# facebookresearch/any4

Measured on AMD Instinct MI355X. Metric: any4 W4A16 GEMM achieved GB/s (m=1, n=k=4096, g=128), higher is better.
Workload: dtype bf16

## Files before the change

any4_amd/csrc/tg_common.cuh:

```cuda
#pragma once
#include <hip/hip_runtime.h>
#include <stdint.h>
#include <stdlib.h>
#include <string.h>
#include <atomic>
#include <type_traits>
#include <utility>

#include "../../include/tinygemm_hip.h"
#include "tg_trace.cuh"

struct GemmParams {
  const char* x;
  const char* w;
  const char* qinfo;
  const char* lut;
  char* y;
  int32_t m, wrows, k;
  int32_t ntiles;
  int32_t ksuper;
  int32_t gshift;
  int32_t ngroups;
  int32_t qtype;
  int32_t rowtiles;
// ... 144 lines not shown

struct BF16 {
  static __device__ __forceinline__ float to_f32(uint16_t h) { return u2f(((uint32_t)h) << 16); }
  static __device__ __forceinline__ float lo_f32(uint32_t pair) { return u2f(pair << 16); }
  static __device__ __forceinline__ float hi_f32(uint32_t pair) { return u2f(pair & 0xffff0000u); }
  static __device__ __forceinline__ uint32_t pack2(float a, float b) {
    f32x2 v = {a, b};
    return __builtin_bit_cast(uint32_t, __builtin_convertvector(v, bf16x2));
  }
  static __device__ __forceinline__ uint16_t from_f32(float a) { return (uint16_t)(pack2(a, 0.f) & 0xffffu); }
  static __device__ __forceinline__ f32x4 mfma(u32x4 a, u32x4 b, f32x4 c) {
    return __builtin_amdgcn_mfma_f32_16x16x32_bf16(__builtin_bit_cast(bf16x8, a), __builtin_bit_cast(bf16x8, b), c, 0, 0, 0);
  }
};
struct F16 {
  static __device__ __forceinline__ float to_f32(uint16_t h) { return (float)__builtin_bit_cast(_Float16, h); }
  static __device__ __forceinline__ float lo_f32(uint32_t pair) { return to_f32((uint16_t)(pair & 0xffffu)); }
  static __device__ __forceinline__ float hi_f32(uint32_t pair) { return to_f32((uint16_t)(pair >> 16)); }
  static __device__ __forceinline__ uint32_t pack2(float a, float b) {
    f32x2 v = {a, b};
    return __builtin_bit_cast(uint32_t, __builtin_convertvector(v, f16x2));
  }
  static __device__ __forceinline__ uint16_t from_f32(float a) { return (uint16_t)(pack2(a, 0.f) & 0xffffu); }
  static __device__ __forceinline__ f32x4 mfma(u32x4 a, u32x4 b, f32x4 c) {
    return __builtin_amdgcn_mfma_f32_16x16x32_f16(__builtin_bit_cast(f16x8, a), __builtin_bit_cast(f16x8, b), c, 0, 0, 0);
  }
};

template <int... VS, typename F>
int pick(int v, F&& f) {
  int rc = TG_PAIR_NA;
  (void)((v == VS && ((rc = f(std::integral_constant<int, VS>{})), true)) || ...);
  return rc;
}
template <typename F>
int pick_dt(int dt, F&& f) {
  return dt == TG_BF16 ? f(BF16{}) : f(F16{});
}

__device__ const float kMX4Values[16] = {0.0f,  0.5f,  1.0f,  1.5f,  2.0f,  3.0f,  4.0f,  6.0f,
                                         -0.0f, -0.5f, -1.0f, -1.5f, -2.0f, -3.0f, -4.0f, -6.0f};

template <typename DT>
__device__ __forceinline__ void store_rows4(char* yb, const char* bias, int64_t elem, int rowg, f32x4 acc) {
  u32x2 o = {DT::pack2(acc[0], acc[1]), DT::pack2(acc[2], acc[3])};
  if (bias) {
    const u32x2 bv = *reinterpret_cast<const u32x2*>(bias + (int64_t)rowg * 2);
    o[0] = DT::pack2(DT::lo_f32(o[0]) + DT::lo_f32(bv[0]), DT::hi_f32(o[0]) + DT::hi_f32(bv[0]));
    o[1] = DT::pack2(DT::lo_f32(o[1]) + DT::lo_f32(bv[1]), DT::hi_f32(o[1]) + DT::hi_f32(bv[1]));
  }
  *reinterpret_cast<u32x2*>(yb + elem * 2) = o;
}


__device__ __forceinline__ u32x4 transpose_rows4(u32x4 v) {
  const auto s01 = __builtin_amdgcn_permlane16_swap(v[0], v[1], false, false);
  const auto s23 = __builtin_amdgcn_permlane16_swap(v[2], v[3], false, false);
  const auto t02 = __builtin_amdgcn_permlane32_swap(s01[0], s23[0], false, false);
  const auto t13 = __builtin_amdgcn_permlane32_swap(s01[1], s23[1], false, false);
  return u32x4{t02[0], t13[0], t02[1], t13[1]};
}

struct DeviceScope {
  int prev = -1;
  bool ok = true;
  explicit DeviceScope(int device) {
    if (device < 0) return;
    if (hipGetDevice(&prev) != hipSuccess) { ok = false; return; }
    if (prev != device && hipSetDevice(device) != hipSuccess) ok = false;
    if (prev == device) prev = -1;
  }
  ~DeviceScope() {
    if (prev >= 0) (void)hipSetDevice(prev);
  }
};

inline int launch_status() {
  const hipError_t e = hipGetLastError();
  return e == hipSuccess ? 0 : (int)e;
}

inline bool aligned16(const void* p) { return (reinterpret_cast<uintptr_t>(p) & 15u) == 0; }
inline int64_t cdiv(int64_t a, int64_t b) { return (a + b - 1) / b; }
inline int group_shift(int g) { return g == 32 ? 5 : g == 64 ? 6 : g == 128 ? 7 : 8; }
inline int64_t coltiles(const GemmParams& p) { return cdiv(p.m, 16); }
inline int words_per_lane(const GemmParams& p) { return p.on_right ? p.inner / 2 : p.inner; }

template <typename D, typename F>
auto assign_if_member(D& d, F f, int) -> decltype(f(d)) { f(d); }
template <typename D, typename F>
void assign_if_member(D&, F, long) {}
template <typename D>
void copy_call(D& d, const GemmParams& p) {
#define TG_COPY(f) assign_if_member(d, [&](auto& t) -> decltype((void)(t.f = p.f)) { t.f = p.f; }, 0)
  TG_COPY(x); TG_COPY(w); TG_COPY(qinfo); TG_COPY(lut); TG_COPY(y);
  TG_COPY(m); TG_COPY(wrows); TG_COPY(k); TG_COPY(ntiles); TG_COPY(ksuper); TG_COPY(gshift); TG_COPY(ngroups); TG_COPY(qtype);
  TG_COPY(stride_x); TG_COPY(stride_w); TG_COPY(stride_qinfo); TG_COPY(stride_lut); TG_COPY(stride_y);
  TG_COPY(bias); TG_COPY(stride_bias); TG_COPY(bias_row_stride);
  TG_COPY(norm_w); TG_COPY(norm_eps); TG_COPY(epilogue); TG_COPY(x_tc); TG_COPY(y_tc); TG_COPY(dry);
#undef TG_COPY
}
inline SplitKParams splitk_params(const GemmParams& p, int splitk) {
  SplitKParams kp;
  copy_call(kp, p);
  kp.rowtiles = p.rowtiles;
  kp.splitk = splitk;
  kp.sk_shift = 0;
  while ((1 << kp.sk_shift) < splitk) ++kp.sk_shift;
  return kp;
}

inline bool has_workspace(const GemmParams& p, int64_t need) { return p.ws_query || (p.ws != nullptr && p.ws_bytes >= need); }

template <auto KERN>
int prepare_lds_kernel() {
  static std::atomic<uint64_t> done{0};
  int dev = 0;
  if (hipGetDevice(&dev) != hipSuccess) return TG_E_DEVICE;
  if (dev >= 0 && dev < 64 && ((done.load(std::memory_order_relaxed) >> dev) & 1u)) return 0;
  hipFuncAttributes fa;
  hipError_t e = hipFuncGetAttributes(&fa, reinterpret_cast<const void*>(KERN));
  if (e != hipSuccess) return (int)e;
  if (fa.sharedSizeBytes != 0) return TG_E_INTERNAL;
  e = hipFuncSetAttribute(reinterpret_cast<const void*>(KERN), hipFuncAttributeMaxDynamicSharedMemorySize, 160 * 1024);
  if (e != hipSuccess) return (int)e;
  if (dev >= 0 && dev < 64) done.fetch_or(1ull << dev, std::memory_order_relaxed);
  return 0;
}
template <auto KERN, typename P>
int launch_lds_kernel(dim3 grid, dim3 block, unsigned lds, hipStream_t st, const P& params, bool decline_on_failure) {
  const int prc = prepare_lds_kernel<KERN>();
  if (prc != 0) return decline_on_failure && prc != TG_E_INTERNAL ? (int)TG_PAIR_NA : prc;
  hipLaunchKernelGGL(KERN, grid, block, lds, st, params);
  return launch_status();
}

inline int cu_count() {
  static std::atomic<int> cache[64];
  int dev = 0;
  if (hipGetDevice(&dev) != hipSuccess || dev < 0 || dev >= 64) return 256;
  int v = cache[dev].load(std::memory_order_relaxed);
  if (v > 0) return v;
  if (hipDeviceGetAttribute(&v, hipDeviceAttributeMultiprocessorCount, dev) != hipSuccess || v <= 0) v = 256;
  cache[dev].store(v, std::memory_order_relaxed);
  return v;
}
inline int plan_cu_count(const GemmParams& p) { return p.dry ? 256 : cu_count(); }


#if !defined(TG_DEV) && !defined(TG_DEV_MIN)
#if defined(TG_PAIR_R) || defined(TG_PAIR_MR1) || defined(TG_PAIR_NSG2) || defined(TG_PAIR_MR1_GPS) || defined(TG_PAIR_RA) ||   \
    defined(TG_PAIR_RA1) || defined(TG_PAIR_RB16) || defined(TG_B16_CHUNK) || defined(TG_PAIR_MIN_ITEMS) || defined(TG_XG_CHUNK) || defined(TG_PAIR_WGS) || \
    defined(TG_PAIR_NSG2_M1) || defined(TG_XR_MIN_M) || defined(TG_XR_R) || defined(TG_XR_R8K) || defined(TG_XR_RMX) || defined(TG_PAIR_M1_LEAN) || \
    defined(TG_PAIR_M1_AHEAD)
#error "the TG_PAIR_* / TG_XG_* / TG_B16_* tuning constants can only be overridden in developer builds (-DTG_DEV or -DTG_DEV_MIN)"
#endif
#endif
#ifndef TG_PAIR_R
#define TG_PAIR_R 2
#endif
#ifndef TG_PAIR_MR1
#define TG_PAIR_MR1 1
#endif
#ifndef TG_PAIR_NSG2
#define TG_PAIR_NSG2 1
#endif
#ifndef TG_PAIR_NSG2_M1
#define TG_PAIR_NSG2_M1 1
#endif
#ifndef TG_PAIR_MR1_GPS
#define TG_PAIR_MR1_GPS 1
#endif
#ifndef TG_PAIR_RA
#define TG_PAIR_RA 2
#endif
#ifndef TG_PAIR_RA1
#define TG_PAIR_RA1 1
#endif
#ifndef TG_PAIR_RB16
#define TG_PAIR_RB16 2
#endif
#ifndef TG_B16_CHUNK
#define TG_B16_CHUNK 4
#endif
#ifndef TG_TILE_W8_MIN_M
#define TG_TILE_W8_MIN_M 17
#endif
#ifndef TG_TILE_MIN_M_SPLIT
#define TG_TILE_MIN_M_SPLIT 17
#endif
#ifndef TG_TILE_MIN_M
#define TG_TILE_MIN_M 65
#endif
#ifndef TG_M1_DEFAULT_MFMA
#define TG_M1_DEFAULT_MFMA 0
#endif
#ifndef TG_PAIR_MIN_ITEMS
#define TG_PAIR_MIN_ITEMS 192
#endif
#ifndef TG_XG_CHUNK
#define TG_XG_CHUNK 4
#endif
#ifndef TG_XR_MIN_M
#define TG_XR_MIN_M 2
#endif
#ifndef TG_XR_RMX
#define TG_XR_RMX 8
#endif
#ifndef TG_XR_R8K
#define TG_XR_R8K 2
#endif
#ifndef TG_XR_R
#define TG_XR_R 4
#endif
#ifndef TG_PAIR_M1_LEAN
#define TG_PAIR_M1_LEAN 1
#endif
#ifndef TG_PAIR_M1_AHEAD
#define TG_PAIR_M1_AHEAD 1
#endif
#ifndef TG_PAIR_WGS
#define TG_PAIR_WGS 512
#endif

}
```

any4_amd/csrc/tg_pair.hip:

```cpp
#include "tg_common.cuh"
#ifdef TG_TU_F16
#define TG_TU_DT F16
#define TG_TU_SUF(n) n##_f16
#else
#define TG_TU_DT BF16
#define TG_TU_SUF(n) n##_bf16
#endif
namespace {
#include "w4_gemm_pair.cuh"
template <typename DT, int I, int GPS, int MR, bool QMX, int NSG, bool XG = false, int LA = 0, bool NORM = false, bool M1_MFMA = false>
int launch_pair_k(const GemmParams& p, PairParams& pp, unsigned lds) {
#ifdef TG_DEV_MIN
#ifndef TG_DEV_GPS
#define TG_DEV_GPS 1
#endif
#ifndef TG_DEV_QMX
#define TG_DEV_QMX false
#endif
#ifndef TG_DEV_MR
#define TG_DEV_MR TG_PAIR_MR1
#endif
#ifndef TG_DEV_LA
#define TG_DEV_LA 0
#endif
  if constexpr (!(std::is_same<DT, BF16>::value && I == 4 && GPS == TG_DEV_GPS && MR == TG_DEV_MR && QMX == TG_DEV_QMX && NSG == TG_DEV_MIN && LA == TG_DEV_LA && !NORM)) return TG_PAIR_NA;
  else {
#endif
  if constexpr (QMX && !std::is_same<DT, BF16>::value) return TG_E_DTYPE;
  else {
  constexpr int RING = (QMX && LA == 0) ? TG_PAIR_R : (MR == 1 && NSG == 4 && LA == 0) ? 4 : GPS > 1 ? (LA ? TG_PAIR_RA1 : 1) : LA == 1 ? TG_PAIR_RA : LA == 2 ? TG_PAIR_RB16 : TG_PAIR_R;
  if (p.dry) return TG_PLAN_PAIR;
  const unsigned wgs = (unsigned)(pp.items < TG_PAIR_WGS ? pp.items : TG_PAIR_WGS);
  return launch_lds_kernel<w4_gemm_pair_kernel<DT, I, GPS, MR, QMX, RING, NSG, M1_MFMA, XG, LA, NORM>>(dim3(wgs), dim3(512), lds, p.st, pp, false);
  }
#ifdef TG_DEV_MIN
  }
#endif
}

inline bool pair_lean_call(const GemmParams& p, const PairParams& pp, bool xg) {
  return TG_PAIR_M1_LEAN && TG_PAIR_MR1 == 1 && TG_PAIR_R == 2 && p.m == 1 && !xg && !p.norm_w && !p.bias && !p.epilogue && !p.x_tc && !p.y_tc &&
         p.wrows % 64 == 0 && p.ntiles * 8 == p.wrows && !pp.red_alias && pp.cblocks == 1 && pp.spw % 2 == 0 && p.ksuper % 2 == 0 &&
         p.numerics != TG_NUM_FAST_MFMA;
}
template <typename DT>
int launch_pair_lean(const GemmParams& p, const PairParams& pp, unsigned lds) {
#ifdef TG_DEV_MIN
  if constexpr (!(std::is_same<DT, BF16>::value && TG_DEV_MIN == 2)) return TG_PAIR_NA;
  else {
#endif
  if (p.dry) return p.dry_detail ? (int)TG_PLAN_PAIR_M1_LEAN : (int)TG_PLAN_PAIR;
  PairLeanParams lp;
  copy_call(lp, p);
  lp.spw = pp.spw; lp.lds_x = pp.lds_x; lp.lds_xs = pp.lds_xs; lp.lds_red = pp.lds_red; lp.rblocks = pp.rblocks; lp.items = pp.items;
  const unsigned wgs = (unsigned)(pp.items < TG_PAIR_WGS ? pp.items : TG_PAIR_WGS);
  return launch_lds_kernel<w4_pair_m1_lean_kernel<DT, TG_PAIR_M1_AHEAD != 0>>(dim3(wgs), dim3(512), lds, p.st, lp, false);
#ifdef TG_DEV_MIN
  }
#endif
}

template <typename DT>
int launch_xprep(const GemmParams& p, const PairParams& pp, int ma, int la = 0) {
  XPrepParams xq;
  xq.la = la;
  xq.x = pp.x; xq.xp = const_cast<char*>(pp.xp); xq.xsum = const_cast<char*>(pp.xsum);
  xq.x_tc = pp.x_tc;
  xq.m = pp.m; xq.k = pp.k; xq.ma = ma; xq.cps = p.inner / 2; xq.gshift = pp.gshift; xq.gch_mask = pp.gch_mask;
  xq.ngroups = pp.ngroups; xq.xs_rows = pp.xs_rows;
  xq.stride_x = pp.stride_x; xq.stride_xp = pp.stride_xp; xq.stride_xsum = pp.stride_xsum;
  const int64_t chunks = (int64_t)pp.m * (pp.k / 32);
  hipLaunchKernelGGL(w4_xprep_kernel<DT>, dim3((unsigned)cdiv(chunks, 256), (unsigned)p.batch), dim3(256), 0, p.st, xq);
  return launch_status();
}

template <typename DT, int I, int GPS, bool QMX, int NSG>
int launch_pair_m(const GemmParams& p, PairParams& pp, unsigned lds, bool xg, int mregs) {
  const bool norm = p.norm_w != nullptr;
  const bool m1 = p.m == 1 && TG_PAIR_MR1 == 1 && (QMX || GPS <= TG_PAIR_MR1_GPS);
  if (mregs != 4) return TG_PAIR_NA;
  if constexpr (I == 8) {
    if constexpr (QMX) return TG_PAIR_NA;
    else {
      if (!m1 || norm) return TG_PAIR_NA;
      return xg ? launch_pair_k<DT, I, GPS, 1, false, NSG, true>(p, pp, lds) : launch_pair_k<DT, I, GPS, 1, false, NSG>(p, pp, lds);
    }
  } else {
  if (xg) return m1 ? launch_pair_k<DT, I, GPS, 1, QMX, NSG, true>(p, pp, lds) : launch_pair_k<DT, I, GPS, 4, QMX, NSG, true>(p, pp, lds);
  if (norm) {
    if constexpr (QMX || GPS > 1) return TG_PAIR_NA;
    else {
      return m1 ? launch_pair_k<DT, I, GPS, 1, false, NSG, false, false, true>(p, pp, lds)
                : launch_pair_k<DT, I, GPS, 4, false, NSG, false, false, true>(p, pp, lds);
    }
  }
  if (m1) return launch_pair_k<DT, I, GPS, 1, QMX, NSG>(p, pp, lds);
  return launch_pair_k<DT, I, GPS, 4, QMX, NSG>(p, pp, lds);
  }
}


struct PairGroups {
  int gps, nsg;
};
template <int I>
PairGroups pair_groups(const GemmParams& p, PairParams& pp) {
  const int g = 1 << p.gshift;
  const PairGroups r = {g >= 16 * I ? 1 : (16 * I) / g, g >= 16 * I ? g / (16 * I) : 1};
  const int units = p.ksuper / r.nsg;
  pp.spw = ((units + 7) / 8) * r.nsg;
  pp.nsg_shift = 0;
  while ((1 << pp.nsg_shift) < r.nsg) ++pp.nsg_shift;
  pp.gch_mask = g / 32 - 1;
  return r;
}

inline bool mx4_blocks_fit(const GemmParams& p, const PairParams& pp, int gps) {
  return !(p.ngroups < 16 || p.ngroups % 4 != 0 || ((pp.spw * gps) % 4 != 0 && pp.spw * gps > 12));
}

template <int I, bool QMX>
unsigned pair_lds_plan(const GemmParams& p, PairParams& pp, int x_bytes, bool alias, bool alias_if_large) {
  pp.lds_x = QMX ? 0 : 65536;
  pp.lds_xs = (pp.lds_x + x_bytes + 32 * I + 15) & ~15;
  pp.lds_red = (pp.lds_xs + (QMX ? 0 : p.ngroups * pp.xs_rows * 4) + 15) & ~15;
  unsigned lds = (unsigned)pp.lds_red + (unsigned)(8 * 2 * pp.rused * pp.red_lanes * 4);
  pp.red_alias = alias || (alias_if_large && lds > 80u * 1024u);
  if (pp.red_alias) {
    lds = (unsigned)pp.lds_red;
    pp.lds_red = 0;
  }
  return lds;
}

inline int64_t pair_workspace(const GemmParams& p, PairParams& pp, int xrows) {
  pp.stride_xp = (int64_t)xrows * p.k * 2;
  pp.stride_xsum = ((int64_t)p.ngroups * pp.xs_rows * 4 + 15) & ~(int64_t)15;
  const int64_t need = p.batch * (pp.stride_xp + pp.stride_xsum);
  if (!has_workspace(p, need)) return 0;
  pp.xp = p.ws;
  pp.xsum = p.ws + p.batch * pp.stride_xp;
  return need;
}

template <typename DT, int I, bool QMX>
int launch_pair(GemmParams& p) {
  constexpr int RW = 64;
  const int mregs = p.m <= 8 ? 4 : 16;
  const int ma = 2 * mregs;
  PairParams pp;
  copy_call(pp, p);
  pp.y_tiles = (p.wrows + 15) / 16;
  const auto [gps, nsg] = pair_groups<I>(p, pp);
  const int mrows = p.m < ma ? p.m : ma;
  pp.rused = mrows < 4 ? mrows : mregs;
  pp.xs_rows = mrows <= 4 ? 4 : ma;
  pp.red_lanes = mrows <= 4 ? 32 : 64;
  pp.x_pitch = p.k * 2 + 16;
  unsigned lds = pair_lds_plan<I, QMX>(p, pp, mrows * pp.x_pitch, !QMX && mrows > 4, false);
  if (QMX && !mx4_blocks_fit(p, pp, gps)) return TG_PAIR_NA;
  if (p.norm_w && (QMX || lds > 80u * 1024u || p.m > ma)) return TG_PAIR_NA;
  int64_t need = 0;
  if (lds > 80u * 1024u) {
    if (mregs != 4 || p.m > ma) return TG_PAIR_NA;
    pp.xw_pitch = 32 * I + 16;
    pp.xw_bytes = (I == 2 ? 16 : 8) * pp.xw_pitch;
    lds = pair_lds_plan<I, QMX>(p, pp, 8 * pp.xw_bytes, pp.red_alias, true);
    if (QMX && pp.red_alias) return TG_PAIR_NA;
    if (lds > 80u * 1024u) return TG_PAIR_NA;
    need = pair_workspace(p, pp, p.m);
    if (!need) return TG_PAIR_NA;
  }
  const bool xg = need != 0;
  pp.rblocks = (p.wrows + RW - 1) / RW;
  pp.cblocks = (p.m + ma - 1) / ma;
  const int64_t items = (int64_t)pp.rblocks * pp.cblocks * p.batch;
  if (items > INT32_MAX) return TG_PAIR_NA;
  if (items < TG_PAIR_MIN_ITEMS) return TG_PAIR_NA;
  pp.items = (int32_t)items;
  pp.chunk = items >= (int64_t)TG_PAIR_WGS * TG_XG_CHUNK * 4 ? TG_XG_CHUNK : 1;
  p.ws_need = need;
  if (xg && !p.dry) {
    const int rc = launch_xprep<DT>(p, pp, ma);
    if (rc != 0) return rc;
  }
  if (gps == 1) {
    const bool fixed = TG_PAIR_NSG2 && (TG_PAIR_NSG2_M1 || !(p.m == 1 && TG_PAIR_MR1 == 1));
    if constexpr (I == 4 && !QMX) {
      if (p.numerics == TG_NUM_FAST_MFMA && p.m == 1 && !xg && !p.norm_w && fixed && nsg == TG_PAIR_R)
        return launch_pair_k<DT, I, 1, 1, false, TG_PAIR_R, false, 0, false, true>(p, pp, lds);
    }
    if constexpr (I == 4 && !QMX) {
      if (fixed && nsg == TG_PAIR_R && pair_lean_call(p, pp, xg)) return launch_pair_lean<DT>(p, pp, lds);
    }
    if (fixed && nsg == TG_PAIR_R) return launch_pair_m<DT, I, 1, QMX, TG_PAIR_R>(p, pp, lds, xg, mregs);
    if constexpr (!QMX) {
      if (fixed && p.m == 1 && TG_PAIR_MR1 == 1 && !p.norm_w && (nsg == 1 || nsg == 4)) {
        if (nsg == 1) return xg ? launch_pair_k<DT, I, 1, 1, false, 1, true>(p, pp, lds) : launch_pair_k<DT, I, 1, 1, false, 1>(p, pp, lds);
        if constexpr (I <= 4)
          return xg ? launch_pair_k<DT, I, 1, 1, false, 4, true>(p, pp, lds) : launch_pair_k<DT, I, 1, 1, false, 4>(p, pp, lds);
      }
    }
    return launch_pair_m<DT, I, 1, QMX, 0>(p, pp, lds, xg, mregs);
  }
  if constexpr (I >= 4) {
    if (gps == 2) return launch_pair_m<DT, I, 2, QMX, 0>(p, pp, lds, xg, mregs);
  }
  if constexpr (I >= 8) {
// ... 69 lines not shown
```

any4_amd/csrc/w4_gemm_pair.cuh:

```cuda
#pragma once
#include "w4_helpers.cuh"
#include "pair_walk.h"

struct PairParams {
  const char* x;
  const char* w;
  const char* qinfo;
  const char* lut;
  char* y;
  int32_t m, wrows, k;
  int32_t ntiles;
  int32_t ksuper;
  int32_t gshift;
  int32_t ngroups;
  int32_t qtype;
  int32_t spw;
  int32_t nsg_shift;
  int32_t gch_mask;
  int32_t x_pitch;
  int32_t lds_x;
  int32_t lds_xs;
  int32_t lds_red;
  int32_t rused;
  int32_t xs_rows;
  int32_t red_lanes;
  int32_t red_alias;
  int32_t rblocks;
  int32_t cblocks;
  int32_t items;
  int64_t stride_x, stride_w, stride_qinfo, stride_lut, stride_y;
  const char* bias;
  int64_t stride_bias;
  int64_t bias_row_stride;
  const char* norm_w;
  float norm_eps;
  int32_t epilogue;
  int32_t dry;
  const char* xp;
  const char* xsum;
  int64_t stride_xp, stride_xsum;
  int32_t xw_pitch;
  int32_t xw_bytes;
  int32_t chunk;
  int32_t x_tc, y_tc;
  int32_t y_tiles;
};

template <typename DT, int I, int GPS, int MR, bool QMX, int R, int NSG = 0, bool M1_MFMA = false, bool XG = false, int LAY = 0, bool NORM = false>
__global__ void __launch_bounds__(512, 4) w4_gemm_pair_kernel(const PairParams p) {
  constexpr bool LA = LAY == 1, LB = LAY == 2, T16 = LAY != 0;
  constexpr bool DOT = !M1_MFMA && MR == 1 && !T16 && (QMX || NSG > 0);
  constexpr bool MXC = QMX;
  static_assert(!NORM || (!XG && !T16 && !QMX), "fused RMSNorm: the workgroup stages the whole activation block itself");
  constexpr int WAVES = 8;
  constexpr int TILES = 2;
  constexpr int WT = LA ? 1 : TILES;
  constexpr int RW = T16 ? 32 : 32 * TILES;
  static_assert(!T16 || (XG && MR == 4 && (LB || I == 2 || I == 4)), "16x16x32 tiles: workspace activations, one pass of up to 16 rows");
  constexpr int NW = LB ? I / 2 : I;
  using acc_t = typename std::conditional<T16, f32x4, f32x16>::type;
  constexpr int CPS = I / 2;
  constexpr int CPG = CPS / GPS;
  constexpr int MREGS = MR == 1 ? 4 : MR;
  constexpr int RF = MR;
  constexpr int MA = T16 ? 16 : 2 * MREGS;
  constexpr int NXW = T16 ? I / 2 : XG ? (MA * 2 * I + 63) / 64 : 1;
  static_assert(!XG || MR <= 4, "XG: one pass is at most 8 activation rows");

  constexpr uint32_t lds0 = 0u;
  const uint32_t lds_x = lds0 + (uint32_t)p.lds_x;
  const uint32_t lds_xs = lds0 + (uint32_t)p.lds_xs;
  const uint32_t lds_red = lds0 + (uint32_t)p.lds_red;

  const int tid = threadIdx.x;
  const int lane = tid & 63;
  const int wave = __builtin_amdgcn_readfirstlane(tid >> 6);
  const int c = lane & 31;
  const int h = lane >> 5;
  const int xa = DOT ? 0 : T16 ? lane & 15 : c;
  const int xq = T16 ? lane >> 4 : 2 * h;
  const int hh = T16 ? lane >> 4 : h;
  auto wrow_local = [&](int t) -> int { return LA ? 16 * ((lane & 15) >> 3) + (lane & 7) + 8 * t : LB ? 16 * t + (lane & 15) : t * 32 + c; };
  const int tcol = tid & 63;
  const int tcol_row = LA ? 16 * ((tcol & 15) >> 3) + (tcol & 7) + 8 * (tcol >> 5) : LB ? 16 * (tcol >> 5) + (tcol & 15) : tcol;

  constexpr bool RR = XG;
  const int chunk = RR ? p.chunk : 1;
  const int it_stride = RR ? (int)gridDim.x * chunk - (chunk - 1) : 1;
  const int it_begin = RR ? (int)blockIdx.x * chunk : (int)(((int64_t)blockIdx.x * p.items) / gridDim.x);
  const int it_end = RR ? p.items : (int)(((int64_t)(blockIdx.x + 1) * p.items) / gridDim.x);
  const int per_problem = p.rblocks * p.cblocks;

  const int s_begin = wave * p.spw;
  const int nl = max(min(p.spw, p.ksuper - s_begin), 0);

  struct Item {
    int b, ct, rb;
  };
  auto decode = [&](int it) -> Item {
    const int b = it / per_problem, r = it - b * per_problem;
    const int ct = r / p.rblocks;
    return Item{b, ct, r - ct * p.rblocks};
  };
  const int adv_b = it_stride / per_problem, adv_r = it_stride - adv_b * per_problem;
  auto advance = [&](const Item& e, bool big) -> Item {
    int b = e.b + (big ? adv_b : 0), r = e.ct * p.rblocks + e.rb + (big ? adv_r : 1);
    if (r >= per_problem) { r -= per_problem; ++b; }
    const int ct = p.cblocks == 1 ? 0 : r / p.rblocks;
    return Item{b, ct, r - ct * p.rblocks};
  };

  uint32_t lp[8];
  auto lut_const = [&]() {
#pragma unroll
    for (int e = 0; e < 16; e += 2) {
      float v0, v1;
      if (p.qtype == TG_Q_INT4) {
        v0 = (float)(e - 8);
        v1 = (float)(e - 7);
      } else {
        const int e1 = e + 1;
        v0 = (e & 8 ? -1.f : 1.f) * ((e & 7) < 5 ? 0.5f * (e & 7) : ((e & 7) == 5 ? 3.f : (e & 7) == 6 ? 4.f : 6.f));
        v1 = (e1 & 8 ? -1.f : 1.f) * ((e1 & 7) < 5 ? 0.5f * (e1 & 7) : ((e1 & 7) == 5 ? 3.f : (e1 & 7) == 6 ? 4.f : 6.f));
      }
      lp[e >> 1] = DT::pack2(v0, v1);
    }
  };
  const bool lut_loaded = p.qtype == TG_Q_ANY4_GLOBAL || p.qtype == TG_Q_ANY4_ROWWISE;
  auto lut_request = [&](const Item& e) {
    const int lrow = min(e.rb * RW + tcol_row, p.wrows - 1);
    const char* lsrc = p.lut + (int64_t)e.b * p.stride_lut + (p.qtype == TG_Q_ANY4_ROWWISE ? (int64_t)lrow * 32 : 0);
    const u32x4 l0 = reinterpret_cast<const u32x4*>(lsrc)[0];
    const u32x4 l1 = reinterpret_cast<const u32x4*>(lsrc)[1];
#pragma unroll
    for (int j = 0; j < 4; ++j) { lp[j] = l0[j]; lp[4 + j] = l1[j]; }
  };

  struct Slot {
    uint32_t w[WT][I];
    uint32_t q[TILES][GPS];
    u32x4 xw[NXW];
  };
  Slot ring[R];
  struct Rows {
    uint32_t wbase[WT];
    uint32_t qrow[TILES];
    uint32_t qrow4[TILES];
    const char* wb;
    const char* qb;
    const char* xpb;
    uint32_t xblk;
    uint32_t xoff[NXW];
  };
  auto rows_of = [&](const Item& e) -> Rows {
    Rows r;
// ... 469 lines not shown
      }
    };

    const int rounds = max((nl + R - 1) / R, 1);
    int l0 = 0;
    const int nblk = QMX ? max((nl + EBS - 1) / EBS, 1) : 1;
    for (int blk = 0; blk < nblk; ++blk) {
      const bool lastb = blk + 1 == nblk;
      if constexpr (QMX) {
#pragma unroll
        for (int t = 0; t < TILES; ++t) ecur[t] = enext[t];
        ebase = eoff_next - blk * 16;
        e_request(lastb ? rnext : rcur, lastb ? 0 : blk + 1, lastb ? has_next && nl > 0 : true);
      }
      const int rend = lastb ? rounds - 1 : (blk + 1) * (EBS / R);
      for (int rd = l0 / R; rd < rend; ++rd, l0 += R) {
#pragma unroll
        for (int j = 0; j < R; ++j) {
          consume(s_begin + l0 + j, ring[j], j);
          issue(rcur, s_begin + l0 + j + R, ring[j], l0 + j + R < nl, NSG == 0 || j % NSG == 0);
        }
      }
    }
#pragma unroll
    for (int j = 0; j < R; ++j) {
      if (l0 + j < nl) consume(s_begin + l0 + j, ring[j], j);
      issue(rnext, s_begin + j, ring[j], has_next && j < nl, NSG == 0 || j % NSG == 0);
    }
    if constexpr (MXC) {
#pragma unroll
      for (int t = 0; t < TILES; ++t)
#pragma unroll
        for (int r = 0; r < RF; ++r) yacc[t][r] = DOT ? dacc[t] : acc[t][r];
    } else if (pending || GPS > 1 || NSG > 0) finalize();
    if constexpr (DOT) {
#pragma unroll
      for (int t = 0; t < TILES; ++t) yacc[t][0] += __shfl_xor(yacc[t][0], 32);
    }

    if (p.red_alias) __syncthreads();
#pragma unroll
    for (int t = 0; t < TILES; ++t) {
#pragma unroll
      for (int r = 0; r < RF; ++r)
        if (r < p.rused && lane < p.red_lanes)
          *(lds_fptr)(lds_red + (uint32_t)((((wave * TILES + t) * p.rused + r) * p.red_lanes + lane) * 4)) = yacc[t][r];
    }
    __syncthreads();
    {
      char* yb = p.y + (int64_t)cur.b * p.stride_y;
      static_assert(TILES == 2, "the output index split below assumes two tiles");
      const int rl_shift = p.red_lanes == 64 ? 6 : 5;
      for (int o = tid; o < TILES * p.rused * p.red_lanes; o += 512) {
        const int l = o & (p.red_lanes - 1), q = o >> rl_shift;
        const int t = q >= p.rused ? 1 : 0, r = q - t * p.rused;
        const int a = T16 ? r + 4 * (l >> 4) : (r & 3) + 8 * (r >> 2) + 4 * (l >> 5);
        const int row = row0 + (LA ? 16 * ((l & 15) >> 3) + (l & 7) + 8 * t : LB ? 16 * t + (l & 15) : t * 32 + (l & 31));
        if (a < mrows && row < p.wrows) {
          float sum = 0.f;
#pragma unroll
          for (int w = 0; w < WAVES; ++w) sum += *(lds_fptr)(lds_red + (uint32_t)((((w * TILES + t) * p.rused + r) * p.red_lanes + l) * 4));
          if (!T16 && p.epilogue == TG_EPI_SWIGLU) {
            if ((l & 15) < 8) {
              float up = 0.f;
#pragma unroll
              for (int w = 0; w < WAVES; ++w) up += *(lds_fptr)(lds_red + (uint32_t)((((w * TILES + t) * p.rused + r) * p.red_lanes + l + 8) * 4));
              *reinterpret_cast<uint16_t*>(yb + ((int64_t)(a0 + a) * (p.wrows >> 1) + ((row >> 4) << 3) + (row & 7)) * 2) = swiglu16<DT>(sum, up);
            }
            continue;
          }
          uint16_t o16 = DT::from_f32(sum);
          if (p.bias)
            o16 = DT::from_f32(DT::lo_f32(o16) + DT::lo_f32(*reinterpret_cast<const uint16_t*>(p.bias + (int64_t)cur.b * p.stride_bias + ((int64_t)(a0 + a) * p.bias_row_stride + row) * 2)));
          *reinterpret_cast<uint16_t*>(yb + (p.y_tc ? tc_a_index(a0 + a, row, p.y_tiles) : (int64_t)(a0 + a) * p.wrows + row) * 2) = o16;
        }
      }
    }
    if (p.red_alias) __syncthreads();
    rcur = rnext;
  }
}

struct XPrepParams {
  const char* x;
  char* xp;
  char* xsum;
  int32_t m, k, ma, cps, gshift, gch_mask, ngroups, xs_rows;
  int32_t la;
  int32_t x_tc;
  int64_t stride_x, stride_xp, stride_xsum;
};

template <typename DT>
__global__ void __launch_bounds__(256) w4_xprep_kernel(const XPrepParams p) {
  const int nch = p.k >> 5;
  const int xi = blockIdx.x * 256 + threadIdx.x;
  const bool on = xi < p.m * nch;
  const int a = on ? xi / nch : 0, ch = on ? xi - a * nch : 0;
  const int b = blockIdx.y;
  uint32_t d[16];
#pragma unroll
  for (int j = 0; j < 16; ++j) d[j] = 0u;
  if (on && p.x_tc) {
    tc_a_load_chunk(p.x + (int64_t)b * p.stride_x, a, ch, p.k >> 4, d);
  } else if (on) {
    const u32x4* src = reinterpret_cast<const u32x4*>(p.x + (int64_t)b * p.stride_x + ((int64_t)a * p.k + ch * 32) * 2);
#pragma unroll
    for (int j = 0; j < 4; ++j) {
      const u32x4 v = src[j];
      d[4 * j] = v[0]; d[4 * j + 1] = v[1]; d[4 * j + 2] = v[2]; d[4 * j + 3] = v[3];
    }
  }
  const int ct = a / p.ma, ar = a - ct * p.ma;
  const int rows = min(p.m - ct * p.ma, p.ma);
  if (on) {
    const int s = ch / p.cps, jc = ch - s * p.cps;
    char* dst = p.xp + (int64_t)b * p.stride_xp + (int64_t)ct * p.ma * p.k * 2 +
                (p.la ? ((int64_t)ch * 4 * (rows + 1) + ar) * 16 : ((int64_t)(s * rows + ar) * p.cps + jc) * 64);
    const int qstride = p.la ? rows + 1 : 1;
#pragma unroll
    for (int q = 0; q < 4; ++q) {
      u32x4 o;
      o[0] = __builtin_amdgcn_perm(d[q + 4], d[q], 0x05040100u);
      o[1] = __builtin_amdgcn_perm(d[q + 12], d[q + 8], 0x05040100u);
      o[2] = __builtin_amdgcn_perm(d[q + 4], d[q], 0x07060302u);
      o[3] = __builtin_amdgcn_perm(d[q + 12], d[q + 8], 0x07060302u);
      reinterpret_cast<u32x4*>(dst)[q * qstride] = o;
    }
    if (p.la && ar == 0)
#pragma unroll
      for (int q = 0; q < 4; ++q) reinterpret_cast<u32x4*>(dst)[q * qstride + rows] = u32x4{0, 0, 0, 0};
  }
  float sum = 0.f;
#pragma unroll
  for (int j = 0; j < 16; ++j) sum = dot2_ones<DT>(d[j], sum);
  for (int o = 1; o <= p.gch_mask; o <<= 1) sum += __shfl_xor(sum, o);
  if (on && (ch & p.gch_mask) == 0)
    reinterpret_cast<float*>(p.xsum + (int64_t)b * p.stride_xsum)[((int64_t)ct * p.ngroups + (ch >> (p.gshift - 5))) * p.xs_rows + ar] = sum;
}

struct PairLeanParams {
  const char* x;
  const char* w;
  const char* qinfo;
  const char* lut;
  char* y;
  int32_t wrows, k, ksuper, qtype;
  int32_t spw;
  int32_t lds_x, lds_xs, lds_red;
  int32_t rblocks, items;
  int64_t stride_x, stride_w, stride_qinfo, stride_lut, stride_y;
};

template <typename DT, bool AHEAD>
__global__ void __launch_bounds__(512, 4) w4_pair_m1_lean_kernel(const PairLeanParams p) {
  constexpr int R = 2, CPS = 2, TILES = 2, WAVES = 8;
  const int tid = threadIdx.x;
  const int lane = tid & 63;
  const int wave = __builtin_amdgcn_readfirstlane(tid >> 6);
  const int c = lane & 31;
  const int h = lane >> 5;
  const uint32_t lds_x = (uint32_t)p.lds_x, lds_xs = (uint32_t)p.lds_xs, lds_red = (uint32_t)p.lds_red;

  int it_begin, it_end;
  pair_walk_range((int)blockIdx.x, (int)gridDim.x, p.items, it_begin, it_end);
  if (it_begin >= it_end) return;
  const int s_begin = wave * p.spw;
  const int nl = max(min(p.spw, p.ksuper - s_begin), 0);

  PairWalkGeom geo;
  geo.rblocks = p.rblocks;
  geo.step[PW_W] = (int64_t)p.ksuper * 2048;
  geo.step[PW_Q] = 256;
  geo.step[PW_LUT] = p.qtype == TG_Q_ANY4_ROWWISE ? 2048 : 0;
  geo.stride[PW_W] = p.stride_w; geo.stride[PW_Q] = p.stride_qinfo; geo.stride[PW_LUT] = p.stride_lut;

  uint32_t wlane = (uint32_t)(((c >> 3) * p.ksuper * 32 + 4 * (c & 7) + 2 * h) * 8);
  uint32_t qlane = (uint32_t)(c * 4);
  const uint32_t llane = p.qtype == TG_Q_ANY4_ROWWISE ? (uint32_t)((tid & 63) * 32) : 0u;
  const int tcol = tid & 63;
  auto pin = [](uint32_t& v) -> uint32_t { asm volatile("" : "+v"(v)); return v; };
  auto uni = [](uint32_t v) -> uint32_t { return (uint32_t)__builtin_amdgcn_readfirstlane((int)v); };

  uint32_t lp[8];
  const bool lut_loaded = p.qtype != TG_Q_INT4;
  auto lut_request = [&](const PairWalk& e) {
    const char* lsrc = p.lut + e.off[PW_LUT] + llane;
    const u32x4 l0 = reinterpret_cast<const u32x4*>(lsrc)[0];
    const u32x4 l1 = reinterpret_cast<const u32x4*>(lsrc)[1];
#pragma unroll
    for (int j = 0; j < 4; ++j) { lp[j] = l0[j]; lp[4 + j] = l1[j]; }
  };

  struct Slot {
    uint32_t w[TILES][4];
    uint32_t q[TILES];
  };
  Slot ring[R];
  auto issue = [&](const PairWalk& e, int s, Slot& sl, bool valid, bool needq) {
    const uint32_t sv = valid ? (uint32_t)s : 0u;
    const char* wb = p.w + e.off[PW_W];
    const char* qb = p.qinfo + e.off[PW_Q];
#pragma unroll
    for (int t = 0; t < TILES; ++t) {
      const char* src = wb + uni(sv * 256u + (uint32_t)(t * p.ksuper * 1024)) + pin(wlane);
      const u32x4 v = __builtin_nontemporal_load(reinterpret_cast<const u32x4*>(src));
#pragma unroll
      for (int j = 0; j < 4; ++j) sl.w[t][j] = v[j];
      if (needq) sl.q[t] = *reinterpret_cast<const uint32_t*>(qb + uni((sv >> 1) * (uint32_t)p.wrows * 4u) + pin(qlane) + t * 128);
    }
  };

  const int nch = p.k >> 5;
  auto x_load = [&](const char* xb, int ch, uint32_t (&d)[16]) {
    const u32x4* src = reinterpret_cast<const u32x4*>(xb + (int64_t)ch * 64);
#pragma unroll
    for (int j = 0; j < 4; ++j) {
      const u32x4 v = src[j];
      d[4 * j] = v[0]; d[4 * j + 1] = v[1]; d[4 * j + 2] = v[2]; d[4 * j + 3] = v[3];
    }
  };
  auto x_store = [&](int ch, bool on, const uint32_t (&d)[16]) {
    if (on) {
      const uint32_t dst = lds_x + (uint32_t)(ch * 64);
#pragma unroll
      for (int q = 0; q < 4; ++q) {
        u32x4 o;
        o[0] = __builtin_amdgcn_perm(d[q + 4], d[q], 0x05040100u);
        o[1] = __builtin_amdgcn_perm(d[q + 12], d[q + 8], 0x05040100u);
        o[2] = __builtin_amdgcn_perm(d[q + 4], d[q], 0x07060302u);
        o[3] = __builtin_amdgcn_perm(d[q + 12], d[q + 8], 0x07060302u);
        *(lds_u32x4ptr)(dst + (uint32_t)(q * 16)) = o;
      }
    }
    float sum = 0.f;
#pragma unroll
    for (int j = 0; j < 16; ++j) sum = dot2_ones<DT>(d[j], sum);
    sum += __shfl_xor(sum, 1);
    sum += __shfl_xor(sum, 2);
    if (on && (ch & 3) == 0) *(lds_fptr)(lds_xs + (uint32_t)((ch >> 2) * 16)) = sum;
  };
  auto x_stage = [&](const char* xb, bool pre, uint32_t (&xd)[16]) {
    for (int it0 = 0; it0 < nch; it0 += 512) {
      const int ch = it0 + tid;
      const bool on = ch < nch;
      if (!(pre && it0 == 0)) {
#pragma unroll
        for (int j = 0; j < 16; ++j) xd[j] = 0u;
        if (on) x_load(xb, ch, xd);
      }
      x_store(on ? ch : 0, on, xd);
    }
  };

  PairWalk cur = pair_walk_first(geo, it_begin);
  if (lut_loaded) lut_request(cur);
  else {
#pragma unroll
    for (int e = 0; e < 16; e += 2) lp[e >> 1] = DT::pack2((float)(e - 8), (float)(e - 7));
  }
  int staged_b = cur.b;
  uint32_t xd0[16];
#pragma unroll
  for (int j = 0; j < 16; ++j) xd0[j] = 0u;
  if (tid < nch) x_load(p.x + (int64_t)cur.b * p.stride_x, tid, xd0);
#pragma unroll
  for (int j = 0; j < R; ++j) {
    __builtin_amdgcn_sched_barrier(0);
    issue(cur, s_begin + j, ring[j], j < nl, j == 0);
  }
  __builtin_amdgcn_sched_barrier(0);
  x_stage(p.x + (int64_t)cur.b * p.stride_x, true, xd0);

  uint32_t colreg[TILES];
#pragma unroll
  for (int t = 0; t < TILES; ++t) colreg[t] = (uint32_t)((t * 32 + c) * 4);
  const uint32_t xrow = lds_x + (uint32_t)(32 * h);

  int table_b = -1;
  for (int it = it_begin; it < it_end; ++it) {
    const bool has_next = it + 1 < it_end;
    PairWalk next = cur;
    if (has_next) pair_walk_next(geo, next);

    if (it == it_begin || p.qtype == TG_Q_ANY4_ROWWISE || (p.qtype == TG_Q_ANY4_GLOBAL && cur.b != table_b)) {
      table_b = cur.b;
      int wv = wave;
      asm volatile("" : "+s"(wv));
      uint32_t hw = lp[0];
#pragma unroll
      for (int j = 1; j < 8; ++j) hw = (wv == j) ? lp[j] : hw;
      const lds_u32ptr tb = (lds_u32ptr)(uint32_t)(wave * 2 * 16 * 256 + tcol * 4);
#pragma unroll
      for (int a = 0; a < 16; ++a) {
        tb[a * 64] = __builtin_amdgcn_perm(hw, lp[a >> 1], (a & 1) ? 0x05040302u : 0x05040100u);
        tb[(16 + a) * 64] = __builtin_amdgcn_perm(hw, lp[a >> 1], (a & 1) ? 0x07060302u : 0x07060100u);
      }
    }
    if (cur.b != staged_b) {
      staged_b = cur.b;
      uint32_t xd[16];
      x_stage(p.x + (int64_t)cur.b * p.stride_x, false, xd);
    }
    if (lut_loaded) lut_request(next);
    __syncthreads();

    float dacc[TILES] = {0.f, 0.f}, prev[TILES] = {0.f, 0.f}, yacc[TILES] = {0.f, 0.f};
    float gs[TILES] = {0.f, 0.f}, gz[TILES] = {0.f, 0.f}, xsv = 0.f;
    auto group_start = [&](const Slot& sl, uint32_t xs_addr) {
#pragma unroll
      for (int t = 0; t < TILES; ++t) {
        const float d = dacc[t] - prev[t];
        prev[t] = dacc[t];
        yacc[t] = __builtin_fmaf(gz[t], xsv, __builtin_fmaf(gs[t], d, yacc[t]));
      }
#pragma unroll
      for (int t = 0; t < TILES; ++t) {
        gs[t] = DT::lo_f32(sl.q[t]);
        gz[t] = h ? 0.f : DT::hi_f32(sl.q[t]);
      }
      xsv = *(lds_cfptr)(xs_addr);
    };
    struct Look {
      u32x4 xf;
      uint32_t bf[TILES][4];
    };
    auto look = [&](const Slot& sl, uint32_t xst, int u, Look& o) {
      const int jc = u >> 1, qq = u & 1;
      o.xf = *(lds_cu32x4ptr)(xst + (uint32_t)(jc * 64 + 16 * qq));
#pragma unroll
      for (int t = 0; t < TILES; ++t) {
        const uint32_t w = sl.w[t][qq * CPS + jc];
#pragma unroll
        for (int j = 0; j < 4; ++j) o.bf[t][j] = *(lds_cu32ptr)(__builtin_amdgcn_perm(w, colreg[t], 0x0c0c0400u + ((uint32_t)j << 8)));
      }
    };
    auto products = [&](const Look& o) {
#pragma unroll
      for (int t = 0; t < TILES; ++t)
#pragma unroll
        for (int j = 0; j < 4; ++j) dacc[t] = dot2<DT>(o.bf[t][j], o.xf[j], dacc[t]);
    };

    const int rounds = __builtin_amdgcn_readfirstlane(max(nl / R, 1));
    uint32_t xst = xrow + (uint32_t)(s_begin * CPS * 64);
    uint32_t xs_addr = lds_xs + (uint32_t)(s_begin * 8);
    if constexpr (!AHEAD) {
      auto round = [&](int l0, bool last) {
#pragma unroll
        for (int j = 0; j < R; ++j) {
          if (l0 + j < nl) {
#pragma unroll
            for (int u = 0; u < 2 * CPS; ++u) {
              Look o;
              look(ring[j], xst + (uint32_t)(j * CPS * 64), u, o);
              __builtin_amdgcn_sched_barrier(0);
              if (j == 0 && u == 0) group_start(ring[0], xs_addr);
              products(o);
              __builtin_amdgcn_sched_barrier(0);
            }
          }
          if (last) issue(next, s_begin + j, ring[j], has_next && j < nl, j == 0);
          else issue(cur, s_begin + l0 + j + R, ring[j], l0 + j + R < nl, j == 0);
        }
      };
      int l0 = 0;
      for (int rd = 0; rd < rounds - 1; ++rd, l0 += R, xst += R * CPS * 64, xs_addr += 16) round(l0, false);
      round(l0, true);
    } else {
      Look la[2];
      auto round = [&](int l0, bool last) {
#pragma unroll
        for (int v = 0; v < 4 * R; ++v) {
          if (v == 0) group_start(ring[0], xs_addr);
          if (v + 1 < 4 * R) look(ring[(v + 1) >> 2], xst + (uint32_t)(((v + 1) >> 2) * CPS * 64), (v + 1) & 3, la[(v + 1) & 1]);
          else if (!last) look(ring[0], xst + (uint32_t)(R * CPS * 64), 0, la[0]);
          if ((v & 3) == 2) {
            const int j = v >> 2;
            if (last) issue(next, s_begin + j, ring[j], has_next, j == 0);
            else issue(cur, s_begin + l0 + j + R, ring[j], true, j == 0);
          }
          products(la[v & 1]);
          __builtin_amdgcn_sched_barrier(0);
        }
      };
      if (nl > 0) {
        look(ring[0], xst, 0, la[0]);
        __builtin_amdgcn_sched_barrier(0);
        int l0 = 0;
        for (int rd = 0; rd < rounds - 1; ++rd, l0 += R, xst += R * CPS * 64, xs_addr += 16) round(l0, false);
        round(l0, true);
      } else {
#pragma unroll
        for (int j = 0; j < R; ++j) issue(next, s_begin + j, ring[j], false, j == 0);
      }
    }
#pragma unroll
    for (int t = 0; t < TILES; ++t) {
      const float d = dacc[t] - prev[t];
      yacc[t] = __builtin_fmaf(gz[t], xsv, __builtin_fmaf(gs[t], d, yacc[t]));
      yacc[t] += __shfl_xor(yacc[t], 32);
    }

    if (lane < 32) {
#pragma unroll
      for (int t = 0; t < TILES; ++t) *(lds_fptr)(lds_red + (uint32_t)(((wave * TILES + t) * 32 + lane) * 4)) = yacc[t];
    }
    __syncthreads();
    if (tid < 64) {
      float sum = 0.f;
#pragma unroll
      for (int w = 0; w < WAVES; ++w) sum += *(lds_fptr)(lds_red + (uint32_t)((w * 64 + tid) * 4));
      *reinterpret_cast<uint16_t*>(p.y + (int64_t)cur.b * p.stride_y + (cur.rb * 64 + tid) * 2) = DT::from_f32(sum);
    }
    cur = next;
  }
}
```

Baseline: 6770.

## Hold activations in registers and broadcast via DPP dot2 for k=4096 lean kernel

Adds a specialised m=1 lean-kernel variant for ksuper=64, spw=8 (k=4096). It loads each wave's activation slice from LDS into 32 registers once per batch and feeds v_dot2c DPP quad_perm instructions, which broadcast the x values across lanes. This replaces the per-step LDS vector loads of x, and fixed compile-time sizes allow full unrolling. The cost is higher register pressure, hand-written asm with s_nop hazards, and a path that only fires for this exact shape.

```diff
diff --git a/any4_amd/csrc/pair_xreg.h b/any4_amd/csrc/pair_xreg.h
--- /dev/null
+++ b/any4_amd/csrc/pair_xreg.h
@@ -0,0 +1,13 @@
+#pragma once
+#include "pair_walk.h"
+
+enum {
+  PAIR_XREG_KSUPER = 64,
+  PAIR_XREG_SPW = 8,
+  PAIR_XREG_STEPS = 32,
+  PAIR_XREG_SLICE_BYTES = 1024
+};
+
+TG_WALK_FN uint32_t pair_xreg_offset(int s, int lane) {
+  return (uint32_t)((s >> 2) * 128 + ((s >> 1) & 1) * 64 + (s & 1) * 16 + (lane >> 5) * 32 + (lane & 3) * 4);
+}
diff --git a/any4_amd/csrc/tg_common.cuh b/any4_amd/csrc/tg_common.cuh
--- a/any4_amd/csrc/tg_common.cuh
+++ b/any4_amd/csrc/tg_common.cuh
@@ -320,7 +320,7 @@
 #if defined(TG_PAIR_R) || defined(TG_PAIR_MR1) || defined(TG_PAIR_NSG2) || defined(TG_PAIR_MR1_GPS) || defined(TG_PAIR_RA) ||   \
     defined(TG_PAIR_RA1) || defined(TG_PAIR_RB16) || defined(TG_B16_CHUNK) || defined(TG_PAIR_MIN_ITEMS) || defined(TG_XG_CHUNK) || defined(TG_PAIR_WGS) || \
     defined(TG_PAIR_NSG2_M1) || defined(TG_XR_MIN_M) || defined(TG_XR_R) || defined(TG_XR_R8K) || defined(TG_XR_RMX) || defined(TG_PAIR_M1_LEAN) || \
-    defined(TG_PAIR_M1_AHEAD)
+    defined(TG_PAIR_M1_AHEAD) || defined(TG_PAIR_M1_XREG)
 #error "the TG_PAIR_* / TG_XG_* / TG_B16_* tuning constants can only be overridden in developer builds (-DTG_DEV or -DTG_DEV_MIN)"
 #endif
 #endif
@@ -387,6 +387,9 @@
 #ifndef TG_PAIR_M1_AHEAD
 #define TG_PAIR_M1_AHEAD 1
 #endif
+#ifndef TG_PAIR_M1_XREG
+#define TG_PAIR_M1_XREG 1
+#endif
 #ifndef TG_PAIR_WGS
 #define TG_PAIR_WGS 512
 #endif
diff --git a/any4_amd/csrc/tg_pair.hip b/any4_amd/csrc/tg_pair.hip
--- a/any4_amd/csrc/tg_pair.hip
+++ b/any4_amd/csrc/tg_pair.hip
@@ -54,6 +54,10 @@
   copy_call(lp, p);
   lp.spw = pp.spw; lp.lds_x = pp.lds_x; lp.lds_xs = pp.lds_xs; lp.lds_red = pp.lds_red; lp.rblocks = pp.rblocks; lp.items = pp.items;
   const unsigned wgs = (unsigned)(pp.items < TG_PAIR_WGS ? pp.items : TG_PAIR_WGS);
+  if constexpr (TG_PAIR_M1_XREG != 0 && TG_PAIR_M1_AHEAD != 0) {
+    if (p.ksuper == PAIR_XREG_KSUPER && pp.spw == PAIR_XREG_SPW)
+      return launch_lds_kernel<w4_pair_m1_lean_kernel<DT, true, true>>(dim3(wgs), dim3(512), lds, p.st, lp, false);
+  }
   return launch_lds_kernel<w4_pair_m1_lean_kernel<DT, TG_PAIR_M1_AHEAD != 0>>(dim3(wgs), dim3(512), lds, p.st, lp, false);
 #ifdef TG_DEV_MIN
   }
diff --git a/any4_amd/csrc/w4_gemm_pair.cuh b/any4_amd/csrc/w4_gemm_pair.cuh
--- a/any4_amd/csrc/w4_gemm_pair.cuh
+++ b/any4_amd/csrc/w4_gemm_pair.cuh
@@ -1,6 +1,7 @@
 #pragma once
 #include "w4_helpers.cuh"
 #include "pair_walk.h"
+#include "pair_xreg.h"
 
 struct PairParams {
   const char* x;
@@ -776,8 +777,28 @@
   int64_t stride_x, stride_w, stride_qinfo, stride_lut, stride_y;
 };
 
-template <typename DT, bool AHEAD>
+template <typename DT, int J>
+__device__ __forceinline__ float dot2_quad(uint32_t xq, uint32_t b, float acc) {
+  static_assert(J >= 0 && J < 4, "a lane of the quad");
+#define TG_DOT2_QUAD(OP, Q) asm(OP " %0, %1, %2 quad_perm:[" #Q "," #Q "," #Q "," #Q "] row_mask:0xf bank_mask:0xf" : "+v"(acc) : "v"(xq), "v"(b))
+  if constexpr (std::is_same<DT, BF16>::value) {
+    if constexpr (J == 0) TG_DOT2_QUAD("v_dot2c_f32_bf16_dpp", 0);
+    else if constexpr (J == 1) TG_DOT2_QUAD("v_dot2c_f32_bf16_dpp", 1);
+    else if constexpr (J == 2) TG_DOT2_QUAD("v_dot2c_f32_bf16_dpp", 2);
+    else TG_DOT2_QUAD("v_dot2c_f32_bf16_dpp", 3);
+  } else {
+    if constexpr (J == 0) TG_DOT2_QUAD("v_dot2c_f32_f16_dpp", 0);
+    else if constexpr (J == 1) TG_DOT2_QUAD("v_dot2c_f32_f16_dpp", 1);
+    else if constexpr (J == 2) TG_DOT2_QUAD("v_dot2c_f32_f16_dpp", 2);
+    else TG_DOT2_QUAD("v_dot2c_f32_f16_dpp", 3);
+  }
+#undef TG_DOT2_QUAD
+  return acc;
+}
+
+template <typename DT, bool AHEAD, bool XREG = false>
 __global__ void __launch_bounds__(512, 4) w4_pair_m1_lean_kernel(const PairLeanParams p) {
+  static_assert(!XREG || AHEAD, "the k = 4096 flavour looks up one step ahead");
   constexpr int R = 2, CPS = 2, TILES = 2, WAVES = 8;
   const int tid = threadIdx.x;
   const int lane = tid & 63;
@@ -789,17 +810,18 @@
   int it_begin, it_end;
   pair_walk_range((int)blockIdx.x, (int)gridDim.x, p.items, it_begin, it_end);
   if (it_begin >= it_end) return;
-  const int s_begin = wave * p.spw;
-  const int nl = max(min(p.spw, p.ksuper - s_begin), 0);
+  const int ksuper = XREG ? (int)PAIR_XREG_KSUPER : p.ksuper, spw = XREG ? (int)PAIR_XREG_SPW : p.spw, kk = XREG ? PAIR_XREG_KSUPER * 64 : p.k;
+  const int s_begin = wave * spw;
+  const int nl = max(min(spw, ksuper - s_begin), 0);
 
   PairWalkGeom geo;
   geo.rblocks = p.rblocks;
-  geo.step[PW_W] = (int64_t)p.ksuper * 2048;
+  geo.step[PW_W] = (int64_t)ksuper * 2048;
   geo.step[PW_Q] = 256;
   geo.step[PW_LUT] = p.qtype == TG_Q_ANY4_ROWWISE ? 2048 : 0;
   geo.stride[PW_W] = p.stride_w; geo.stride[PW_Q] = p.stride_qinfo; geo.stride[PW_LUT] = p.stride_lut;
 
-  uint32_t wlane = (uint32_t)(((c >> 3) * p.ksuper * 32 + 4 * (c & 7) + 2 * h) * 8);
+  uint32_t wlane = (uint32_t)(((c >> 3) * ksuper * 32 + 4 * (c & 7) + 2 * h) * 8);
   uint32_t qlane = (uint32_t)(c * 4);
   const uint32_t llane = p.qtype == TG_Q_ANY4_ROWWISE ? (uint32_t)((tid & 63) * 32) : 0u;
   const int tcol = tid & 63;
@@ -827,7 +849,7 @@
     const char* qb = p.qinfo + e.off[PW_Q];
 #pragma unroll
     for (int t = 0; t < TILES; ++t) {
-      const char* src = wb + uni(sv * 256u + (uint32_t)(t * p.ksuper * 1024)) + pin(wlane);
+      const char* src = wb + uni(sv * 256u + (uint32_t)(t * ksuper * 1024)) + pin(wlane);
       const u32x4 v = __builtin_nontemporal_load(reinterpret_cast<const u32x4*>(src));
 #pragma unroll
       for (int j = 0; j < 4; ++j) sl.w[t][j] = v[j];
@@ -835,7 +857,7 @@
     }
   };
 
-  const int nch = p.k >> 5;
+  const int nch = kk >> 5;
   auto x_load = [&](const char* xb, int ch, uint32_t (&d)[16]) {
     const u32x4* src = reinterpret_cast<const u32x4*>(xb + (int64_t)ch * 64);
 #pragma unroll
@@ -901,6 +923,8 @@
   for (int t = 0; t < TILES; ++t) colreg[t] = (uint32_t)((t * 32 + c) * 4);
   const uint32_t xrow = lds_x + (uint32_t)(32 * h);
 
+  [[maybe_unused]] uint32_t X[XREG ? PAIR_XREG_STEPS : 1];
+  [[maybe_unused]] int xreg_b = -1;
   int table_b = -1;
   for (int it = it_begin; it < it_end; ++it) {
     const bool has_next = it + 1 < it_end;
@@ -928,6 +952,14 @@
     }
     if (lut_loaded) lut_request(next);
     __syncthreads();
+    if constexpr (XREG) {
+      if (cur.b != xreg_b) {
+        xreg_b = cur.b;
+        const uint32_t xbase = lds_x + (uint32_t)(wave * PAIR_XREG_SLICE_BYTES);
+#pragma unroll
+        for (int s = 0; s < PAIR_XREG_STEPS; ++s) X[s] = *(lds_cu32ptr)(xbase + pair_xreg_offset(s, lane));
+      }
+    }
 
     float dacc[TILES] = {0.f, 0.f}, prev[TILES] = {0.f, 0.f}, yacc[TILES] = {0.f, 0.f};
     float gs[TILES] = {0.f, 0.f}, gz[TILES] = {0.f, 0.f}, xsv = 0.f;
@@ -969,7 +1001,54 @@
     const int rounds = __builtin_amdgcn_readfirstlane(max(nl / R, 1));
     uint32_t xst = xrow + (uint32_t)(s_begin * CPS * 64);
     uint32_t xs_addr = lds_xs + (uint32_t)(s_begin * 8);
-    if constexpr (!AHEAD) {
+    if constexpr (XREG) {
+      struct LookB {
+        uint32_t bf[TILES][4];
+      };
+      auto lookb = [&](const Slot& sl, int u, LookB& o) {
+        const int jc = u >> 1, qq = u & 1;
+#pragma unroll
+        for (int t = 0; t < TILES; ++t) {
+          const uint32_t w = sl.w[t][qq * CPS + jc];
+#pragma unroll
+          for (int j = 0; j < 4; ++j) o.bf[t][j] = *(lds_cu32ptr)(__builtin_amdgcn_perm(w, colreg[t], 0x0c0c0400u + ((uint32_t)j << 8)));
+        }
+      };
+      auto productsx = [&](const LookB& o, uint32_t xq) {
+#pragma unroll
+        for (int t = 0; t < TILES; ++t) {
+          dacc[t] = dot2_quad<DT, 0>(xq, o.bf[t][0], dacc[t]);
+          dacc[t] = dot2_quad<DT, 1>(xq, o.bf[t][1], dacc[t]);
+          dacc[t] = dot2_quad<DT, 2>(xq, o.bf[t][2], dacc[t]);
+          dacc[t] = dot2_quad<DT, 3>(xq, o.bf[t][3], dacc[t]);
+        }
+      };
+      auto settle = [&]() { asm volatile("s_nop 2" : "+v"(dacc[0]), "+v"(dacc[1])); };
+      constexpr int ROUNDS = PAIR_XREG_SPW / R;
+      LookB la[2];
+      lookb(ring[0], 0, la[0]);
+      __builtin_amdgcn_sched_barrier(0);
+#pragma unroll
+      for (int rd = 0; rd < ROUNDS; ++rd) {
+#pragma unroll
+        for (int v = 0; v < 4 * R; ++v) {
+          if (v == 0) {
+            if (rd > 0) settle();
+            group_start(ring[0], xs_addr + (uint32_t)(rd * 16));
+          }
+          if (v + 1 < 4 * R) lookb(ring[(v + 1) >> 2], (v + 1) & 3, la[(v + 1) & 1]);
+          else if (rd + 1 < ROUNDS) lookb(ring[0], 0, la[0]);
+          if ((v & 3) == 2) {
+            const int j = v >> 2;
+            if (rd + 1 < ROUNDS) issue(cur, s_begin + rd * R + j + R, ring[j], true, j == 0);
+            else issue(next, s_begin + j, ring[j], true, j == 0);
+          }
+          productsx(la[v & 1], X[rd * 4 * R + v]);
+          __builtin_amdgcn_sched_barrier(0);
+        }
+      }
+      settle();
+    } else if constexpr (!AHEAD) {
       auto round = [&](int l0, bool last) {
 #pragma unroll
         for (int j = 0; j < R; ++j) {
```

After: 6735. No clear change (-0.5%).
